# sozoluffy/TensorNetworks

Hardware: AMD Instinct MI355X
Metric: ksd_gradient_steps_per_sec (higher is better)
Workload: dtype f64; 1 GPU; n16_L6_dense; n_qubits=16, layers=6, ansatz=hardware_efficient, params=288, gram=dense, bayesian_network=synthetic n=16 seed=0 (SURVEY 8d), optimizer=adam lr=0.005 cosine clip=10, parallelism=paramshift + gram row shard x1

## Files before the change

tensornetworks_amd/csrc/plan.cpp:

```cpp
#include "plan.hpp"

#include <algorithm>
#include <array>
#include <cstring>
#include <utility>

namespace bornvi {

int num_params(int ansatz, int n, int layers) {
  if (ansatz == 0 || ansatz == 1) return layers * 3 * n;
  if (ansatz == 2) return layers * 2 * n;
  return -1;
}

bool build_gate_list(int ansatz, int n, int layers, std::vector<Gate>& g) {
  g.clear();
  int p = 0;
  auto rot = [&](int kind, int w) { g.push_back({kind, w, -1, p++}); };
  if (ansatz == 0) {
    for (int i = 0; i < n; ++i) g.push_back({G_H, i, -1, -1});
    for (int l = 0; l < layers; ++l) {
      for (int i = 0; i < n; ++i) { rot(G_RX, i); rot(G_RY, i); rot(G_RZ, i); }
      if (n > 1) {
        for (int i = 0; i + 1 < n; ++i) g.push_back({G_CNOT, i, i + 1, -1});
        if (n > 2) g.push_back({G_CNOT, n - 1, 0, -1});
        if (l % 2 == 0 && n > 2)
          for (int i = 0; i < n - 2; i += 2) g.push_back({G_CZ, i, i + 2, -1});
      }
    }
  } else if (ansatz == 1) {
    for (int i = 0; i < n; ++i) g.push_back({G_H, i, -1, -1});
    for (int l = 0; l < layers; ++l) {
      for (int i = 0; i < n; ++i) { rot(G_RX, i); rot(G_RY, i); rot(G_RZ, i); }
      if (n > 1)
        for (int i = 0; i < n; ++i)
          for (int j = i + 1; j < n; ++j) g.push_back({G_CZ, i, j, -1});
    }
  } else if (ansatz == 2) {
    for (int l = 0; l < layers; ++l) {
      for (int i = 0; i < n; ++i) { rot(G_RY, i); rot(G_RZ, i); }
      if (n > 1) {
        for (int i = 0; i + 1 < n; ++i) g.push_back({G_CNOT, i, i + 1, -1});
        if (n > 2) g.push_back({G_CNOT, n - 1, 0, -1});
      }
    }
  } else {
    return false;
  }
  return true;
}

namespace {

enum { K_U1 = 0, K_CX = 1, K_CZ = 2 };
struct Op { int kind, a, b, idx; };
using Fused = std::array<uint32_t, FUSED_WORDS>;

void fuse_gates(const std::vector<Gate>& gates, int n, std::vector<Op>& ops, std::vector<Fused>& fused) {
  std::vector<int> open(n, -1);
  for (const Gate& g : gates) {
    if (g.kind <= G_RZ) {
      int f = open[g.w0];
      if (f < 0 || fused[f][1] >= (uint32_t)FUSED_MAX_ELEMS) {
        Fused nf; nf.fill(0xffffffffu);
        nf[0] = (uint32_t)g.w0; nf[1] = 0;
        fused.push_back(nf);
        f = (int)fused.size() - 1;
        open[g.w0] = f;
        ops.push_back({K_U1, g.w0, -1, f});
      }
      uint32_t e = fused[f][1]++;
      fused[f][2 + 2 * e] = (uint32_t)g.kind;
      fused[f][3 + 2 * e] = (uint32_t)g.param;
    } else {
      open[g.w0] = open[g.w1] = -1;
      ops.push_back({g.kind == G_CNOT ? K_CX : K_CZ, g.w0, g.w1, -1});
    }
  }
}

inline int op_target(const Op& o) { return o.kind == K_U1 ? o.a : (o.kind == K_CX ? o.b : -1); }

void greedy_select(const std::vector<Op>& ops, const std::vector<int>& pool, int n, int cap,
                   std::vector<int>& sel, std::vector<int>& rest, std::vector<int>& targets) {
  std::vector<char> blocked(n, 0), in_t(n, 0);
  sel.clear(); rest.clear(); targets.clear();
  for (int idx : pool) {
    const Op& o = ops[idx];
    bool blk = blocked[o.a] || (o.b >= 0 && blocked[o.b]);
    int t = op_target(o);
    if (!blk && t >= 0 && !in_t[t]) {
      if ((int)targets.size() < cap) { in_t[t] = 1; targets.push_back(t); }
      else blk = true;
    }
    if (blk) {
      blocked[o.a] = 1;
      if (o.b >= 0) blocked[o.b] = 1;
      rest.push_back(idx);
    } else {
      sel.push_back(idx);
    }
  }
}

int fixed_select(const std::vector<Op>& ops, const std::vector<int>& pool, int n, const std::vector<char>& allowed,
                 std::vector<int>& sel, std::vector<int>& rest, std::vector<int>& targets) {
  std::vector<char> blocked(n, 0), in_t(n, 0);
  sel.clear(); rest.clear(); targets.clear();
  int bound_ops = 0;
  for (int idx : pool) {
    const Op& o = ops[idx];
    bool blk = blocked[o.a] || (o.b >= 0 && blocked[o.b]);
    const int t = op_target(o);
    if (!blk && t >= 0 && !allowed[t]) blk = true;
    if (blk) {
      blocked[o.a] = 1;
      if (o.b >= 0) blocked[o.b] = 1;
      rest.push_back(idx);
    } else {
      if (t >= 0) { ++bound_ops; if (!in_t[t]) { in_t[t] = 1; targets.push_back(t); } }
      sel.push_back(idx);
    }
  }
  return bound_ops;
}

void choose_pass(const std::vector<Op>& ops, const std::vector<int>& pool, int n, int k, std::vector<int>& sel,
                 std::vector<int>& rest, std::vector<int>& targets) {
  std::vector<std::vector<char>> cands;
  {
    std::vector<int> s, r, t;
    greedy_select(ops, pool, n, k, s, r, t);
    std::vector<char> a(n, 0);
    for (int w : t) a[w] = 1;
    int cnt = (int)t.size();
    for (int w = n - 1; w >= 0 && cnt < k; --w) if (!a[w]) { a[w] = 1; ++cnt; }
    cands.push_back(a);
  }
  if (k < n)
    for (int s0 = 0; s0 < n; ++s0) {
      std::vector<char> a(n, 0);
      for (int j = 0; j < k; ++j) a[(s0 + j) % n] = 1;
      cands.push_back(a);
    }
  long best_score = -1;
  std::vector<int> s1, r1, t1, s2, r2, t2;
  for (const auto& a : cands) {
    const int here = fixed_select(ops, pool, n, a, s1, r1, t1);
    if (s1.empty()) continue;
    int next_best = 0;
    if (!r1.empty() && k < n)
      for (const auto& a2 : cands) {
        const int nb = fixed_select(ops, r1, n, a2, s2, r2, t2);
        if (nb > next_best) next_best = nb;
      }
    const long score = (long)(here + next_best) * 4096 + (long)s1.size();
    if (score > best_score) { best_score = score; sel = s1; rest = r1; targets = t1; }
  }
  if (best_score < 0) greedy_select(ops, pool, n, k, sel, rest, targets);
}

struct StageSel {
  std::vector<int> pre_cx, pre_cz, us, post_cx, post_cz, targets;
  size_t count() const { return pre_cx.size() + pre_cz.size() + us.size() + post_cx.size() + post_cz.size(); }
};

void stage_select(const std::vector<Op>& ops, const std::vector<int>& pool, int n, int cap, StageSel& S,
                  std::vector<int>& rest, bool defer_cx3 = false, bool read_map = false) {
  std::vector<char> blocked(n, 0), in_t(n, 0), has_u(n, 0);
  std::vector<int> wphase(n, 0);
  rest.clear();
  for (int idx : pool) {
    const Op& o = ops[idx];
    bool blk = blocked[o.a] || (o.b >= 0 && blocked[o.b]);
    int ph = -1;
    if (!blk) {
      const int mx = std::max(wphase[o.a], o.b >= 0 ? wphase[o.b] : 0);
      if (o.kind == K_U1) ph = (mx <= 1 && !has_u[o.a]) ? 2 : -1;
      else if (o.kind == K_CX) ph = mx <= 0 ? 0 : (mx <= 3 ? 3 : -1);
      else ph = mx <= 1 ? 1 : (mx <= 4 ? 4 : -1);
      if (ph < 0) blk = true;
    }
    const int t = op_target(o);
    if (!blk && t >= 0 && !in_t[t] && !(read_map && o.kind == K_CX && ph == 0)) {
      if (defer_cx3 && o.kind == K_CX) blk = true;
      else if ((int)S.targets.size() < cap) { in_t[t] = 1; S.targets.push_back(t); }
      else blk = true;
    }
    if (blk) {
      blocked[o.a] = 1;
      if (o.b >= 0) blocked[o.b] = 1;
      rest.push_back(idx);
      continue;
    }
    wphase[o.a] = std::max(wphase[o.a], ph);
    if (o.b >= 0) wphase[o.b] = std::max(wphase[o.b], ph);
    switch (ph) {
      case 0: S.pre_cx.push_back(idx); break;
      case 1: S.pre_cz.push_back(idx); break;
      case 2: S.us.push_back(idx); has_u[o.a] = 1; break;
      case 3: S.post_cx.push_back(idx); break;
      default: S.post_cz.push_back(idx); break;
    }
  }
}

std::vector<int> order_for_banks(std::vector<int> pos) {
  std::sort(pos.begin(), pos.end());
  std::vector<int> out;
  std::vector<char> used(pos.size(), 0);
  bool res_used[4] = {false, false, false, false};
  auto take = [&](auto pred) -> bool {
    for (size_t i = 0; i < pos.size(); ++i)
      if (!used[i] && pred(pos[i])) { used[i] = 1; out.push_back(pos[i]); res_used[pos[i] & 3] = true; return true; }
    return false;
  };
  for (int s = 0; s < 3 && out.size() < pos.size(); ++s)
    if (!take([&](int p) { return (p & 3) != 3 && !res_used[p & 3]; }))
      take([&](int) { return true; });
  if (out.size() < pos.size())
    if (!take([&](int p) { return (p & 3) == 3; })) take([&](int) { return true; });
  if (out.size() < pos.size() && out.size() >= 2) {
    int r0 = out[0] & 3, r1 = out[1] & 3;
    if (!take([&](int p) { return (p & 3) == r0 || (p & 3) == r1; })) take([&](int) { return true; });
  }
  for (size_t i = 0; i < pos.size(); ++i)
    if (!used[i]) out.push_back(pos[i]);
  return out;
}

void split_pass_ops(const std::vector<Op>& ops, const std::vector<int>& pass_ops, int n, bool is_init,
                    std::vector<int>& lead, std::vector<int>& core, std::vector<int>& trail) {
  lead.clear(); core.clear(); trail.clear();
  std::vector<char> touched(n, 0);
  std::vector<int> mid;
  for (int idx : pass_ops) {
    const Op& o = ops[idx];
    if (!is_init && o.kind == K_CX && !touched[o.a] && !touched[o.b]) { lead.push_back(idx); continue; }
    touched[o.a] = 1; if (o.b >= 0) touched[o.b] = 1;
    mid.push_back(idx);
  }
  std::fill(touched.begin(), touched.end(), 0);
  std::vector<int> trail_rev, core_rev;
  for (size_t q = mid.size(); q-- > 0;) {
    const Op& o = ops[mid[q]];
    if (o.kind == K_CX && !touched[o.a] && !touched[o.b]) { trail_rev.push_back(mid[q]); continue; }
    touched[o.a] = 1; if (o.b >= 0) touched[o.b] = 1;
    core_rev.push_back(mid[q]);
  }
  core.assign(core_rev.rbegin(), core_rev.rend());
  trail.assign(trail_rev.rbegin(), trail_rev.rend());
}

int count_stages(const std::vector<Op>& ops, const std::vector<int>& core, int n, int r, bool defer_cx3, bool read_map) {
  std::vector<int> pool = core, rest;
  int cnt = 0;
  while (!pool.empty()) {
    StageSel sel;
    stage_select(ops, pool, n, r, sel, rest, defer_cx3, read_map);
    if (sel.count() == 0) return 1 << 20;
    ++cnt;
    pool = rest;
  }
  return cnt;
}
bool pick_defer_policy(const std::vector<Op>& ops, const std::vector<int>& core, int n, int r, bool read_map) {
  return read_map && count_stages(ops, core, n, r, true, true) < count_stages(ops, core, n, r, false, true);
}

void first_last_stage_targets(const std::vector<Op>& ops, const std::vector<int>& pass_ops, int n, int r, bool is_init,
                              std::vector<int>& first_t, std::vector<int>& last_t, bool read_map) {
  std::vector<int> lead, core, trail, rest;
  split_pass_ops(ops, pass_ops, n, is_init, lead, core, trail);
  first_t.clear(); last_t.clear();
  std::vector<int> pool = core;
  bool first = true;
  const bool defer = pick_defer_policy(ops, core, n, r, read_map);
  while (!pool.empty()) {
    StageSel sel;
    stage_select(ops, pool, n, r, sel, rest, defer, read_map);
    if (sel.count() == 0) break;
    if (first) { first_t = sel.targets; first = false; }
    last_t = sel.targets;
    pool = rest;
  }
}

struct PassInfo {
  std::vector<int> ops;
  std::vector<int> targets;
  std::vector<int> local;
  std::vector<int> global;
  std::vector<int> lds_wire;
  std::vector<int> in_low;
  std::vector<int> out_low;
};

}

namespace {
struct BuildSpec {
  int n = 0;
  std::vector<Op> ops;
  std::vector<Fused> fused;
  int n_params = 0, n_gates = 0;
  bool in_state = false;
  bool out_state = false;
  std::vector<std::pair<int, int>> out_perm;
};
bool build_plan(const BuildSpec& spec, const PlanOptions& opt, Plan& plan, std::string& msg);
}

namespace {
bool make_plan_impl(int ansatz, int n, int layers, const PlanOptions& opt, Plan& plan, std::string& msg, std::vector<TailOp>* tail);
}

bool make_plan(int ansatz, int n, int layers, const PlanOptions& opt, Plan& plan, std::string& msg) {
  return make_plan_impl(ansatz, n, layers, opt, plan, msg, nullptr);
}

bool make_state_plan(int ansatz, int n, int layers, const PlanOptions& opt, Plan& plan, std::vector<TailOp>& tail, std::string& msg) {
  tail.clear();
  return make_plan_impl(ansatz, n, layers, opt, plan, msg, &tail);
}

namespace {
bool make_plan_impl(int ansatz, int n, int layers, const PlanOptions& opt, Plan& plan, std::string& msg, std::vector<TailOp>* tail) {
  if (n < 1 || n > MAX_PLAN_QUBITS) { msg = "num qubits must be in [1, " + std::to_string(MAX_PLAN_QUBITS) + "]"; return false; }
  if (layers < 0) { msg = "layers must be >= 0"; return false; }
  std::vector<Gate> gates;
  if (!build_gate_list(ansatz, n, layers, gates)) { msg = "unknown ansatz id"; return false; }
  BuildSpec spec;
  spec.n = n;
  fuse_gates(gates, n, spec.ops, spec.fused);
  {
    size_t last_u = spec.ops.size();
    while (last_u > 0 && spec.ops[last_u - 1].kind != K_U1) --last_u;
    for (size_t q = last_u; q < spec.ops.size(); ++q) {
      if (tail) tail->push_back({spec.ops[q].kind == K_CZ ? 1 : 0, spec.ops[q].a, spec.ops[q].b});
      else if (spec.ops[q].kind == K_CX) spec.out_perm.push_back({spec.ops[q].a, spec.ops[q].b});
    }
    spec.ops.resize(last_u);
  }
  spec.out_state = tail != nullptr;
  spec.n_params = num_params(ansatz, n, layers);
  spec.n_gates = (int)gates.size();
  if (opt.kmulti == 0 && n > opt.kmax && opt.kmax >= 13) {
    PlanOptions o11 = opt, o13 = opt;
    o11.kmulti = 11;
    o13.kmulti = 13;
    if (opt.r == 3) return build_plan(spec, o13, plan, msg);
    Plan p13;
    std::string m13;
    if (build_plan(spec, o13, p13, m13)) {
      FastTables ft;
      if ((build_fast_tables(p13, FAST_TABLE_MAX_BYTES, ft) && p13.fast_lds_bytes(ft.max_tab_rows) <= MAX_LDS_BYTES) ||
          n - o11.kmulti > 16) {
        plan = std::move(p13);
        return true;
      }
    }
    return build_plan(spec, o11, plan, msg);
  }
  return build_plan(spec, opt, plan, msg);
}
}

bool make_kron_plan(int n, const PlanOptions& opt, Plan& plan, std::string& msg) {
  if (n < 1 || n > MAX_PLAN_QUBITS) { msg = "num bits must be in [1, " + std::to_string(MAX_PLAN_QUBITS) + "]"; return false; }
  BuildSpec spec;
  spec.n = n;
  Fused f; f.fill(0xffffffffu); f[0] = 0; f[1] = 0;
  spec.fused.push_back(f);
  for (int w = n - 1; w >= 0; --w) spec.ops.push_back({K_U1, w, -1, 0});
  spec.in_state = spec.out_state = true;
  spec.n_gates = n;
  if (opt.kmulti == 0 && n - 12 > 16 && opt.kmax >= 13) {
    PlanOptions o13 = opt;
    o13.kmulti = 13;
    return build_plan(spec, o13, plan, msg);
  }
  return build_plan(spec, opt, plan, msg);
}

namespace {
bool build_plan(const BuildSpec& spec, const PlanOptions& opt, Plan& plan, std::string& msg) {
  const int n = spec.n;
  const std::vector<Op>& ops = spec.ops;
  const std::vector<Fused>& fused = spec.fused;
  const int kmulti = opt.kmulti > 0 ? opt.kmulti : (n <= 16 ? 11 : 12);
  const int k = (n <= opt.kmax) ? n : std::min(opt.kmax, kmulti);
  const int r = std::min(opt.r, k);
  if (r > 4) { msg = "at most 4 register wires"; return false; }
  int threads = 64;
  while (threads < (1 << (k - r))) threads <<= 1;
  if (threads > opt.max_threads) { msg = "tile needs more threads than allowed"; return false; }
  if (fused.size() > 65535) { msg = "too many fused gates"; return false; }

  std::vector<PassInfo> passes;
  {
    std::vector<int> pool(ops.size());
    for (size_t i = 0; i < ops.size(); ++i) pool[i] = (int)i;
    std::vector<int> sel, rest, tg;
    while (!pool.empty()) {
      choose_pass(ops, pool, n, k, sel, rest, tg);
      if (sel.empty()) { msg = "planner made no progress"; return false; }
      PassInfo pi; pi.ops = sel; pi.targets = tg;
      passes.push_back(pi);
      pool = rest;
    }
    if (passes.empty()) passes.push_back(PassInfo{});
  }
  const int lo_can = std::min(opt.lo, k);
  std::vector<int> canon_low;
  for (int p = 0; p < lo_can; ++p) canon_low.push_back(n - 1 - p);
  std::vector<int> canon_low_out = canon_low;
  {
    auto count_with = [&](int lo) {
      std::vector<char> in(n, 0);
      int cnt = 0;
      for (int w : passes.back().targets) { in[w] = 1; ++cnt; }
      for (int p = 0; p < lo; ++p) if (!in[n - 1 - p]) { in[n - 1 - p] = 1; ++cnt; }
      return cnt;
    };
    int lo_fit = -1;
    for (int lo = lo_can; lo >= std::min(3, lo_can); --lo)
      if (count_with(lo) <= k) { lo_fit = lo; break; }
    if (lo_fit < 0) passes.push_back(PassInfo{});
    else canon_low_out.resize(lo_fit);
  }
  if (spec.in_state) {
    std::vector<char> in(n, 0);
    int cnt = 0;
    for (int w : passes.front().targets) { in[w] = 1; ++cnt; }
    for (int w : canon_low) if (!in[w]) { in[w] = 1; ++cnt; }
    if (cnt > k) passes.insert(passes.begin(), PassInfo{});
  }
  const int np = (int)passes.size();
  for (int i = 0; i < np; ++i) {
    PassInfo& P = passes[i];
    std::vector<char> in(n, 0);
    auto add = [&](int w) { if (!in[w] && (int)P.local.size() < k) { in[w] = 1; P.local.push_back(w); } };
    for (int w : P.targets) add(w);
    if (i == np - 1) for (int w : canon_low_out) add(w);
    if (i == 0 && spec.in_state) for (int w : canon_low) add(w);
    if (i + 1 < np) for (int w : passes[i + 1].targets) add(w);
    if (i > 0) for (int w : passes[i - 1].local) add(w);
    for (int w = n - 1; w >= 0; --w) add(w);
    for (int w = 0; w < n; ++w) if (!in[w]) P.global.push_back(w);
  }
  if (spec.in_state) passes[0].in_low = canon_low;
  for (int i = 0; i < np; ++i) {
    PassInfo& P = passes[i];
    std::vector<char> placed(n, 0);
    for (int w : P.in_low) { P.lds_wire.push_back(w); placed[w] = 1; }
    std::vector<int> others;
    for (int w : P.local) if (!placed[w]) others.push_back(w);
    std::sort(others.begin(), others.end());
    for (int w : others) P.lds_wire.push_back(w);
    if (i == np - 1) { P.out_low = canon_low_out; break; }
    std::vector<char> nxt(n, 0);
    for (int w : passes[i + 1].local) nxt[w] = 1;
    std::vector<int> ldspos(n, -1);
    for (int j = 0; j < k; ++j) ldspos[P.lds_wire[j]] = j;
    std::vector<int> pos;
    for (int w : P.local) if (nxt[w]) pos.push_back(ldspos[w]);
    {
      std::vector<int> f_cur, l_cur, f_nxt, l_nxt;
      first_last_stage_targets(ops, P.ops, n, r, i == 0 && !spec.in_state, f_cur, l_cur, opt.use_read_map());
      first_last_stage_targets(ops, passes[i + 1].ops, n, r, false, f_nxt, l_nxt, opt.use_read_map());
      std::vector<char> busy(n, 0);
      for (int w : l_cur) busy[w] = 1;
      for (int w : f_nxt) busy[w] = 1;
      std::vector<int> quiet;
      for (int q : pos) if (!busy[P.lds_wire[q]]) quiet.push_back(q);
      if ((int)quiet.size() >= std::min(4, std::min(opt.lo, k))) pos = quiet;
    }
    pos = order_for_banks(pos);
    const int lo = std::min((int)pos.size(), std::min(opt.lo, k));
    for (int j = 0; j < lo; ++j) P.out_low.push_back(P.lds_wire[pos[j]]);
    passes[i + 1].in_low = P.out_low;
  }
  std::vector<std::vector<int>> layout(np, std::vector<int>(n, -1));
  for (int i = 0; i < np; ++i) {
    if (i == np - 1) { for (int w = 0; w < n; ++w) layout[i][w] = n - 1 - w; continue; }
    int p = 0;
    for (int w : passes[i].out_low) layout[i][w] = p++;
    if (opt.contig_out) {
      std::vector<char> nxt(n, 0);
      for (int w : passes[i + 1].local) nxt[w] = 1;
      for (int w : passes[i].local) if (layout[i][w] < 0 && nxt[w]) layout[i][w] = p++;
      for (int w : passes[i].local) if (layout[i][w] < 0) layout[i][w] = p++;
    }
    for (int w = 0; w < n; ++w) if (layout[i][w] < 0) layout[i][w] = p++;
  }

  std::vector<uint32_t>& W = plan.words;
  plan.max_stages = 0;
  W.assign(PH_SIZE, 0);
  W[PH_MAGIC] = PLAN_MAGIC; W[PH_N] = n; W[PH_K] = k; W[PH_NPASSES] = np;
  W[PH_NFUSED] = (uint32_t)fused.size(); W[PH_NPARAMS] = (uint32_t)spec.n_params;
  W[PH_THREADS] = threads; W[PH_R] = r; W[PH_NGATES] = (uint32_t)spec.n_gates;
  W[PH_OFF_FUSED] = (uint32_t)W.size();
  for (const Fused& f : fused) W.insert(W.end(), f.begin(), f.end());
  W[PH_OFF_PASSTAB] = (uint32_t)W.size();
  W.resize(W.size() + np, 0);
  plan.pass_off.assign(np, 0);

  for (int i = 0; i < np; ++i) {
    const PassInfo& P = passes[i];
    const uint32_t base = (uint32_t)W.size();
    plan.pass_off[i] = base;
    W[W[PH_OFF_PASSTAB] + i] = base;
    W.resize(base + PW_STAGES, 0);
    uint32_t flags = 0;
    if (i == 0 && !spec.in_state) flags |= PASS_INIT;
    if (i == np - 1) flags |= spec.out_state ? PASS_FINAL_STATE : PASS_FINAL;
    std::vector<int> ldspos(n, -1), gpos(n, -1);
    for (int j = 0; j < k; ++j) ldspos[P.lds_wire[j]] = j;
    for (int m = 0; m < n - k; ++m) gpos[P.global[m]] = m;
    auto extpos = [&](int w) { return ldspos[w] >= 0 ? ldspos[w] : k + gpos[w]; };
    const int lo_in = (int)P.in_low.size(), lo_out = (int)P.out_low.size();
    W[base + PW_FLAGS] = flags; W[base + PW_K] = k; W[base + PW_N] = n;
    W[base + PW_LO_IN] = lo_in; W[base + PW_LO_OUT] = lo_out; W[base + PW_THREADS] = threads;
    auto put_byte = [&](int table, int j, int value) { W[base + table + (j >> 2)] |= (uint32_t)value << (8 * (j & 3)); };
    if (k > 16 || n - k > 16) { msg = "tile or workgroup index wider than 16 bits"; return false; }
    for (int j = 0; j < k; ++j) {
      W[base + PW_WIRE_OF_LDS + j] = P.lds_wire[j];
      put_byte(PW_IN_PHYS, j, (i > 0) ? layout[i - 1][P.lds_wire[j]] : (n - 1 - P.lds_wire[j]));
    }
    for (int m = 0; m < n - k; ++m) {
      W[base + PW_WIRE_OF_G + m] = P.global[m];
      put_byte(PW_IN_GPHYS, m, (i > 0) ? layout[i - 1][P.global[m]] : (n - 1 - P.global[m]));
      put_byte(PW_OUT_GPHYS, m, layout[i][P.global[m]]);
    }
    std::vector<int> lead, core, trail;
    split_pass_ops(ops, P.ops, n, (flags & PASS_INIT) != 0, lead, core, trail);
    struct LExpr { uint32_t l, g; };
    auto compose_lin = [&](const std::vector<int>& seq, bool reverse) {
      std::vector<LExpr> ex(k);
      for (int b2 = 0; b2 < k; ++b2) ex[b2] = LExpr{1u << b2, 0u};
      for (size_t q = 0; q < seq.size(); ++q) {
        const Op& o = ops[seq[reverse ? seq.size() - 1 - q : q]];
        const LExpr ce = ldspos[o.a] >= 0 ? ex[ldspos[o.a]] : LExpr{0u, 1u << gpos[o.a]};
        ex[ldspos[o.b]].l ^= ce.l; ex[ldspos[o.b]].g ^= ce.g;
      }
      return ex;
    };
    auto put_half = [&](int table, int j, uint32_t value) { W[base + table + (j >> 1)] |= (value & 0xffffu) << (16 * (j & 1)); };
    {
      const std::vector<LExpr> fin = compose_lin(lead, false);
      for (int j = 0; j < k; ++j) {
        uint32_t col = 0;
        for (int b2 = 0; b2 < k; ++b2) col |= ((fin[b2].l >> j) & 1u) << b2;
        put_half(PW_IN_MASK, j, lds_swizzle(col));
      }
      for (int m = 0; m < n - k; ++m) {
        uint32_t col = 0;
        for (int b2 = 0; b2 < k; ++b2) col |= ((fin[b2].g >> m) & 1u) << b2;
        put_half(PW_IN_GMASK, m, lds_swizzle(col));
      }
    }
    {
      const std::vector<LExpr> fout = compose_lin(trail, true);
      auto out_col = [&](int q) { uint32_t col = 0; for (int b2 = 0; b2 < k; ++b2) col |= ((fout[b2].l >> q) & 1u) << b2; return lds_swizzle(col); };
      std::vector<char> isl(n, 0);
      int j = 0;
      for (int w : P.out_low) { put_half(PW_OUT_MASK, j, out_col(ldspos[w])); put_byte(PW_OUT_PHYS, j, layout[i][w]); isl[w] = 1; ++j; }
      for (int q = 0; q < k; ++q) {
        int w = P.lds_wire[q];
        if (isl[w]) continue;
        put_half(PW_OUT_MASK, j, out_col(q)); put_byte(PW_OUT_PHYS, j, layout[i][w]); ++j;
      }
      for (int m = 0; m < n - k; ++m) {
        uint32_t col = 0;
        for (int b2 = 0; b2 < k; ++b2) col |= ((fout[b2].g >> m) & 1u) << b2;
        put_half(PW_OUT_GMASK, m, lds_swizzle(col));
      }
      std::vector<uint32_t> wire_col(n, 0);
      for (int w = 0; w < n; ++w) wire_col[w] = 1u << layout[i][w];
      if (i == np - 1 && !spec.out_perm.empty()) {
        std::vector<uint32_t> reach(n);
        std::vector<uint32_t> expr(n);
        for (int w = 0; w < n; ++w) expr[w] = 1u << w;
        for (const auto& cx : spec.out_perm) expr[cx.second] ^= expr[cx.first];
        for (int w = 0; w < n; ++w) {
          uint32_t col = 0;
          for (int w2 = 0; w2 < n; ++w2) if ((expr[w2] >> w) & 1u) col ^= 1u << layout[i][w2];
          wire_col[w] = col;
        }
      }
      {
        std::vector<char> isl2(n, 0);
        int j2 = 0;
        for (int w : P.out_low) { W[base + PW_OUT_COL + j2] = wire_col[w]; isl2[w] = 1; ++j2; }
        for (int q = 0; q < k; ++q) {
          const int w = P.lds_wire[q];
          if (isl2[w]) continue;
          W[base + PW_OUT_COL + j2] = wire_col[w]; ++j2;
        }
        for (int m = 0; m < n - k; ++m) W[base + PW_OUT_GCOL + m] = wire_col[P.global[m]];
      }
    }
    std::vector<int> pool = core, rest;
    uint32_t nstages = 0;
    const bool defer_cx3 = pick_defer_policy(ops, core, n, r, opt.use_read_map());
    while (!pool.empty()) {
      StageSel sel;
      stage_select(ops, pool, n, r, sel, rest, defer_cx3, opt.use_read_map());
      if (sel.count() == 0) { msg = "stage planner made no progress"; return false; }
      std::vector<char> isr(n, 0);
      std::vector<int> regw;
      {
        std::vector<char> has_u(n, 0);
        for (int idx : sel.us) has_u[ops[idx].a] = 1;
        for (int w : sel.targets) if (has_u[w]) regw.push_back(w);
        for (int w : sel.targets) if (!has_u[w]) regw.push_back(w);
      }
      for (int w : regw) isr[w] = 1;
      {
        std::vector<char> lowwire(n, 0);
        for (int w : P.in_low) lowwire[w] = 1;
        for (int w : P.out_low) lowwire[w] = 1;
        for (int avoid = 1; avoid >= 0; --avoid)
          for (int j = k - 1; j >= 0 && (int)regw.size() < r; --j)
            if (!isr[P.lds_wire[j]] && !(avoid && lowwire[P.lds_wire[j]])) { isr[P.lds_wire[j]] = 1; regw.push_back(P.lds_wire[j]); }
      }
      std::vector<int> regbit(n, -1);
      uint32_t rho = 0;
      for (int b = 0; b < r; ++b) { regbit[regw[b]] = b; rho |= (uint32_t)ldspos[regw[b]] << (8 * b); }
      std::vector<int> freepos;
      for (int j = 0; j < k; ++j) if (!isr[P.lds_wire[j]]) freepos.push_back(j);
      freepos = order_for_banks(freepos);
      uint32_t io_flags = 0;
      {
        const bool first = (nstages == 0) && !(flags & PASS_INIT);
        const bool last = rest.empty();
        auto lead_with = [&](const std::vector<int>& lowpos) {
          for (int q : lowpos) if (isr[P.lds_wire[q]]) return false;
          std::vector<char> taken(k, 0);
          std::vector<int> others;
          for (int q : lowpos) taken[q] = 1;
          for (int q : freepos) if (!taken[q]) others.push_back(q);
          std::vector<int> ord = lowpos;
          ord.insert(ord.end(), others.begin(), others.end());
          freepos = ord;
          return true;
        };
        if (first && !P.in_low.empty()) {
          std::vector<int> lowpos;
          for (size_t q = 0; q < P.in_low.size(); ++q) lowpos.push_back((int)q);
          if ((int)lowpos.size() <= k - r && lead_with(lowpos)) io_flags |= STAGE_FROM_HBM;
        }
        if (last && !(io_flags & STAGE_FROM_HBM) && !P.out_low.empty()) {
          std::vector<int> lowpos;
          for (int w : P.out_low) lowpos.push_back(ldspos[w]);
          if ((int)lowpos.size() <= k - r && lead_with(lowpos)) io_flags |= STAGE_TO_HBM;
        }
      }
      uint32_t tpos[4] = {0, 0, 0, 0};
      for (size_t j = 0; j < freepos.size() && j < 16; ++j) tpos[j / 4] |= (uint32_t)freepos[j] << (8 * (j % 4));

      struct Expr { uint32_t areg, bext; };
      auto compose = [&](const std::vector<int>& seq, bool reverse, Expr (&ex)[4]) {
        for (int t = 0; t < 4; ++t) ex[t] = Expr{1u << t, 0u};
        for (size_t q = 0; q < seq.size(); ++q) {
          const Op& o = ops[seq[reverse ? seq.size() - 1 - q : q]];
          const int rt = regbit[o.b];
          Expr ce = regbit[o.a] >= 0 ? ex[regbit[o.a]] : Expr{0u, 1u << extpos(o.a)};
          ex[rt].areg ^= ce.areg; ex[rt].bext ^= ce.bext;
        }
      };
      Expr pre[4], post[4];
      compose(sel.post_cx, false, post);
      std::vector<Expr> pre_pos((size_t)k);
      for (int p2 = 0; p2 < k; ++p2) pre_pos[(size_t)p2] = Expr{0u, 1u << p2};
      for (int t = 0; t < r; ++t) pre_pos[(size_t)ldspos[regw[t]]] = Expr{1u << t, 0u};
      for (size_t q = 0; q < sel.pre_cx.size(); ++q) {
        const Op& o = ops[sel.pre_cx[sel.pre_cx.size() - 1 - q]];
        const Expr ce = ldspos[o.a] >= 0 ? pre_pos[(size_t)ldspos[o.a]] : Expr{0u, 1u << extpos(o.a)};
        Expr& te = pre_pos[(size_t)ldspos[o.b]];
        te.areg ^= ce.areg; te.bext ^= ce.bext;
      }
      for (int t = 0; t < 4; ++t) pre[t] = t < r ? pre_pos[(size_t)ldspos[regw[t]]] : Expr{1u << t, 0u};
      auto slot_offset = [&](const Expr (&ex)[4], int j) {
        uint32_t off = 0;
        for (int t = 0; t < r; ++t)
          if (__builtin_popcount(ex[t].areg & (uint32_t)j) & 1) off |= 1u << ldspos[regw[t]];
        return off;
      };
      auto read_slot_offset = [&](int j) {
        uint32_t off = 0;
        for (int p2 = 0; p2 < k; ++p2)
          if (__builtin_popcount(pre_pos[(size_t)p2].areg & (uint32_t)j) & 1) off |= 1u << p2;
        return off;
      };
      auto emit_signq = [&](const std::vector<int>& czs, const Expr (&ex)[4]) {
        uint32_t U[32]; std::memset(U, 0, sizeof(U));
        uint32_t Sym[32]; std::memset(Sym, 0, sizeof(Sym));
        for (int idx : czs) {
          int ea = extpos(ops[idx].a), eb = extpos(ops[idx].b);
          int lo2 = std::min(ea, eb), hi2 = std::max(ea, eb);
          U[lo2] ^= 1u << hi2;
          Sym[lo2] ^= 1u << hi2; Sym[hi2] ^= 1u << lo2;
        }
        for (int a = 0; a < 32; ++a) W.push_back(U[a]);
        uint32_t qbits = 0;
        for (int j = 0; j < 16; ++j) {
          uint32_t off = (j < (1 << r)) ? slot_offset(ex, j) : 0u, m = 0, qv = 0;
          for (int a = 0; a < 32; ++a)
            if (off >> a & 1) { m ^= Sym[a]; qv ^= (uint32_t)__builtin_popcount(off & U[a]) & 1u; }
          W.push_back(m);
          qbits |= qv << j;
        }
        W.push_back(qbits);
      };

      const uint32_t sbase = (uint32_t)W.size();
      W.resize(sbase + STAGE_HDR_WORDS, 0);
      W[sbase + 1] = rho;
      for (int q = 0; q < 4; ++q) W[sbase + 2 + q] = tpos[q];
      uint32_t fidx[4] = {0xffffu, 0xffffu, 0xffffu, 0xffffu};
      for (int idx : sel.us) fidx[regbit[ops[idx].a]] = (uint32_t)ops[idx].idx;
      W[sbase + 6] = fidx[0] | (fidx[1] << 16);
      W[sbase + 7] = fidx[2] | (fidx[3] << 16);
      if (nstages >= (uint32_t)MAX_STAGES) { msg = "too many stages in one pass"; return false; }
      W[base + PW_MATS + 2 * nstages] = W[sbase + 6];
      W[base + PW_MATS + 2 * nstages + 1] = W[sbase + 7];
      for (int t = 0; t < 4; ++t) { W[sbase + 8 + t] = t < r ? pre[t].bext : 0u; W[sbase + 12 + t] = t < r ? post[t].bext : 0u; }
      for (int j = 0; j < 16; ++j) {
        W[sbase + 16 + j] = (j < (1 << r)) ? lds_swizzle(read_slot_offset(j)) : 0u;
        W[sbase + 32 + j] = (j < (1 << r)) ? lds_swizzle(slot_offset(post, j)) : 0u;
      }
      bool cross_read = false;
      for (int p2 = 0; p2 < k; ++p2)
        if (!isr[P.lds_wire[p2]]) {
          W[sbase + 48 + p2] = pre_pos[(size_t)p2].bext ^ (1u << p2);
          if (W[sbase + 48 + p2] || pre_pos[(size_t)p2].areg) cross_read = true;
        }
      uint32_t flags = io_flags | (cross_read ? STAGE_CROSS_READ : 0u);
      Expr ident[4];
      for (int t = 0; t < 4; ++t) ident[t] = Expr{1u << t, 0u};
      if (!sel.pre_cz.empty()) { flags |= STAGE_SIGN_PRE; emit_signq(sel.pre_cz, ident); }
      if (!sel.post_cz.empty()) { flags |= STAGE_SIGN_POST; emit_signq(sel.post_cz, post); }
      for (uint32_t tt = 0; tt < (1u << (k - r)); ++tt) {
        uint32_t bse = 0;
        for (size_t j = 0; j < freepos.size(); ++j) bse |= ((tt >> j) & 1u) << freepos[j];
        W.push_back(lds_swizzle(bse) | (bse << 16));
      }
      const uint32_t nwords = (uint32_t)W.size() - sbase;
      if (nwords >= (1u << 16)) { msg = "stage too large"; return false; }
      W[sbase] = (uint32_t)r | (flags << 8) | (nwords << 16);
      ++nstages;
      pool = rest;
    }
    W[base + PW_NSTAGES] = nstages;
    if ((int)nstages > plan.max_stages) plan.max_stages = (int)nstages;
  }
  W[PH_TOTAL] = (uint32_t)W.size();
  plan.param_first_pass.assign(spec.n_params, np > 0 ? np - 1 : 0);
  std::vector<char> param_seen(spec.n_params, 0);
  for (int i = 0; i < np; ++i) {
    const uint32_t* PWp = W.data() + plan.pass_off[i];
    for (uint32_t sm = 0; sm < PWp[PW_NSTAGES] * 4u; ++sm) {
      const uint32_t w = PWp[PW_MATS + (sm >> 1)];
      const uint32_t f = (sm & 1u) ? (w >> 16) : (w & 0xffffu);
      if (f == 0xffffu) continue;
      const uint32_t* fw = W.data() + W[PH_OFF_FUSED] + f * FUSED_WORDS;
      for (uint32_t e = 0; e < fw[1]; ++e) {
        const uint32_t par = fw[3 + 2 * e];
        if (par != 0xffffffffu && par < (uint32_t)spec.n_params && !param_seen[par]) { param_seen[par] = 1; plan.param_first_pass[par] = i; }
      }
    }
  }
  for (int q = 0; q < spec.n_params; ++q) if (!param_seen[q]) plan.param_first_pass[q] = 0;
  plan.n = n; plan.k = k; plan.r = r; plan.n_passes = np; plan.n_fused = (int)fused.size();
  plan.n_params = spec.n_params; plan.threads = threads; plan.n_gates = spec.n_gates;
  return true;
}
}

bool build_fast_tables(const Plan& plan, size_t max_bytes, FastTables& out) {
  out.words.clear(); out.pass_off.clear(); out.any_sign = false; out.max_tab_rows = 1;
  const int n = plan.n, k = plan.k;
  const int r = plan.r;
  if ((r != 4 && r != 3) || k < (r == 4 ? 10 : 9) || plan.threads != (1 << (k - r)) || n - k > 16) return false;
  out.r = r;
  const int kt = k - r;
  const int nslots = 1 << r;
  const size_t per_stage = (size_t)1 << (n - r);
  size_t total = 0;
  for (int i = 0; i < plan.n_passes; ++i) {
    const uint32_t* P = plan.words.data() + plan.pass_off[i];
    const uint32_t nst = P[PW_NSTAGES];
    if (nst > (uint32_t)MAX_STAGES || nst * 4u * (uint32_t)r > (uint32_t)plan.threads) return false;
    bool any_sign = false;
    const uint32_t* S = P + PW_STAGES;
    for (uint32_t s = 0; s < nst; ++s) { if ((S[0] >> 8) & (STAGE_SIGN_PRE | STAGE_SIGN_POST)) any_sign = true; S += S[0] >> 16; }
    total += FH_WORDS + (size_t)nst * FS_WORDS + (size_t)nst * per_stage * (any_sign ? 2 : 1) + 2 * per_stage;
  }
  if (total * sizeof(uint32_t) > max_bytes || total >= (size_t)0xffffffffu) return false;
  std::vector<uint32_t>& W = out.words;
  W.reserve(total);
  auto parity = [](uint32_t v) { return (uint32_t)__builtin_popcount(v) & 1u; };
  for (int i = 0; i < plan.n_passes; ++i) {
    const uint32_t* P = plan.words.data() + plan.pass_off[i];
    const uint32_t nst = P[PW_NSTAGES];
    const uint32_t hbase = (uint32_t)W.size();
    out.pass_off.push_back(hbase);
    W.resize(hbase + FH_WORDS + (size_t)nst * FS_WORDS, 0);
    uint32_t sign_pre = 0, sign_post = 0;
    {
      const uint32_t* S = P + PW_STAGES;
      for (uint32_t s = 0; s < nst; ++s) {
        const uint32_t sf = (S[0] >> 8) & 0xffu;
        if (sf & STAGE_SIGN_PRE) sign_pre |= 1u << s;
        if (sf & STAGE_SIGN_POST) sign_post |= 1u << s;
        S += S[0] >> 16;
      }
    }
    const bool any_sign = (sign_pre | sign_post) != 0;
    if (any_sign) out.any_sign = true;
    out.max_tab_rows = std::max(out.max_tab_rows, (int)nst + __builtin_popcount(sign_pre | sign_post));
    const uint32_t rw_base = (uint32_t)W.size();
    W.resize(W.size() + (size_t)nst * per_stage, 0);
    const uint32_t sg_base = any_sign ? (uint32_t)W.size() : 0u;
    if (any_sign) W.resize(W.size() + (size_t)nst * per_stage, 0);
    W[hbase + FH_NSTAGES] = nst; W[hbase + FH_RW_BASE] = rw_base; W[hbase + FH_SG_BASE] = sg_base;
    W[hbase + FH_SIGN_PRE] = sign_pre; W[hbase + FH_SIGN_POST] = sign_post;
    const uint32_t* S = P + PW_STAGES;
    for (uint32_t s = 0; s < nst; ++s) {
      const uint32_t hdr = S[0];
      if ((hdr & 0xffu) != (uint32_t)r) { out.words.clear(); out.pass_off.clear(); return false; }
      const uint32_t sflags = (hdr >> 8) & 0xffu, nwords = hdr >> 16, rho = S[1];
      uint32_t* FS = W.data() + hbase + FH_WORDS + (size_t)s * FS_WORDS;
      FS[FS_FI01] = S[6]; FS[FS_FI23] = S[7];
      {
        const uint32_t fi[4] = {S[6] & 0xffffu, S[6] >> 16, S[7] & 0xffffu, S[7] >> 16};
        uint32_t ng = 0;
        while (ng < (uint32_t)r && fi[ng] != 0xffffu) ++ng;
        for (uint32_t b = ng; b < 4; ++b)
          if (fi[b] != 0xffffu) { out.words.clear(); out.pass_off.clear(); return false; }
        FS[FS_KIND] = ng | ((sflags & STAGE_SIGN_PRE) ? 8u : 0u) | ((sflags & STAGE_SIGN_POST) ? 16u : 0u);
        FS[FS_CROSS] = (sflags & STAGE_CROSS_READ) ? 1u : 0u;
        if (!fast_stage_kind_supported(FS[FS_KIND])) { out.words.clear(); out.pass_off.clear(); return false; }
      }
      for (int b = 0; b < r; ++b) { FS[FS_RB + b] = S[16 + (1 << b)] << 4; FS[FS_WB + b] = S[32 + (1 << b)] << 4; }
      for (int j = 0; j < nslots; ++j) {
        uint32_t lr = 0, lw = 0;
        for (int b = 0; b < r; ++b) if (j >> b & 1) { lr ^= S[16 + (1 << b)]; lw ^= S[32 + (1 << b)]; }
        if (lr != S[16 + j] || lw != S[32 + j]) { out.words.clear(); out.pass_off.clear(); return false; }
      }
      uint32_t sri[4] = {0, 0, 0, 0}, rpos[4] = {0, 0, 0, 0};
      for (int b = 0; b < r; ++b) { rpos[b] = (rho >> (8 * b)) & 0xffu; sri[b] = lds_swizzle(1u << rpos[b]); }
      const uint32_t* Qpre = (sflags & STAGE_SIGN_PRE) ? S + STAGE_HDR_WORDS : nullptr;
      const uint32_t* Qpost = (sflags & STAGE_SIGN_POST) ? S + STAGE_HDR_WORDS + (Qpre ? SIGNQ_WORDS : 0) : nullptr;
      const uint32_t* tab = S + STAGE_HDR_WORDS + (Qpre ? SIGNQ_WORDS : 0) + (Qpost ? SIGNQ_WORDS : 0);
      auto sign_bits = [&](const uint32_t* Q, uint32_t e) {
        uint32_t acc = 0;
        for (int q = 0; q < n; ++q) acc ^= ((e >> q) & 1u) & parity(e & Q[q]);
        uint32_t m = 0;
        for (int j = 0; j < 16; ++j) m |= (((Q[48] >> j) ^ acc ^ parity(e & Q[32 + j])) & 1u) << j;
        return m;
      };
      uint32_t* RW = W.data() + rw_base + (size_t)s * per_stage;
      uint32_t* SG = any_sign ? W.data() + sg_base + (size_t)s * per_stage : nullptr;
      for (uint32_t g = 0; g < (1u << (n - k)); ++g)
        for (uint32_t t = 0; t < (1u << kt); ++t) {
          const uint32_t pb = tab[t] & 0xffffu, base = tab[t] >> 16;
          const uint32_t e = base | (g << k);
          uint32_t lflip = 0, sflip = 0, e2 = e;
          for (int b = 0; b < r; ++b) {
            if (parity(e & S[8 + b])) lflip ^= sri[b];
            if (parity(e & S[12 + b])) { sflip ^= sri[b]; e2 |= 1u << rpos[b]; }
          }
          for (int p2 = 0; p2 < k; ++p2)
            if (S[48 + p2] && parity(e & S[48 + p2])) lflip ^= lds_swizzle(1u << p2);
          RW[((size_t)g << kt) + t] = (pb ^ lflip) | ((pb ^ sflip) << 16);
          if (SG) SG[((size_t)g << kt) + t] = (Qpre ? sign_bits(Qpre, e) : 0u) | ((Qpost ? sign_bits(Qpost, e2) : 0u) << 16);
        }
      S += nwords;
    }
    const uint32_t pflags = P[PW_FLAGS];
    const uint32_t kt2 = (uint32_t)kt;
    auto tbyte = [&](int table, int j) { return (P[table + (j >> 2)] >> (8 * (j & 3))) & 0xffu; };
    auto thalf = [&](int table, int j) { return (P[table + (j >> 1)] >> (16 * (j & 1))) & 0xffffu; };
    const uint32_t ksize = 1u << k;
    const uint32_t ngl = 1u << (n - k);
    if (nst > 0) {
      const uint32_t* S0 = P + PW_STAGES;
      const uint32_t* SL = S0;
      for (uint32_t s2 = 0; s2 + 1 < nst; ++s2) SL += SL[0] >> 16;
      const uint32_t f0 = (S0[0] >> 8) & 0xffu, fl = (SL[0] >> 8) & 0xffu;
      std::vector<uint32_t> inv(ksize);
      if ((f0 & STAGE_FROM_HBM) && !(pflags & PASS_INIT)) {
        auto slot_lin = [&](uint32_t u) { uint32_t o = 0; for (int j = 0; j < k; ++j) if (u >> j & 1) o ^= thalf(PW_IN_MASK, j); return o; };
        auto phys_u = [&](uint32_t u) { uint32_t o = 0; for (int j = 0; j < k; ++j) if (u >> j & 1) o |= 1u << tbyte(PW_IN_PHYS, j); return o; };
        for (uint32_t u = 0; u < ksize; ++u) inv[slot_lin(u)] = u;
        const uint32_t tab = (uint32_t)W.size();
        W.resize(W.size() + per_stage, 0);
        const uint32_t* RW0 = W.data() + rw_base;
        bool ok = true;
        uint32_t basis[4] = {0, 0, 0, 0};
        for (int b = 0; b < r; ++b) basis[b] = phys_u(inv[W[hbase + FH_WORDS + FS_RB + b] >> 4]) << 4;
        for (uint32_t g = 0; g < ngl && ok; ++g) {
          uint32_t gslot = 0, gphys = 0;
          for (int m = 0; m < n - k; ++m) if (g >> m & 1) { gslot ^= thalf(PW_IN_GMASK, m); gphys |= 1u << tbyte(PW_IN_GPHYS, m); }
          for (uint32_t t = 0; t < (1u << kt2); ++t) {
            const uint32_t rslot = RW0[((size_t)g << kt2) + t] & 0xffffu;
            const uint32_t off = (phys_u(inv[rslot ^ gslot]) | gphys) << 4;
            W[tab + ((size_t)g << kt2) + t] = off;
          }
// ... 398 lines not shown
```

Before: 236.1 steps/s.

## Let the pass and stage planners commute gates that share diagonal (control/CZ) wires

```diff
diff --git a/tensornetworks_amd/csrc/plan.cpp b/tensornetworks_amd/csrc/plan.cpp
--- a/tensornetworks_amd/csrc/plan.cpp
+++ b/tensornetworks_amd/csrc/plan.cpp
@@ -81,21 +81,31 @@
 
 inline int op_target(const Op& o) { return o.kind == K_U1 ? o.a : (o.kind == K_CX ? o.b : -1); }
 
-void greedy_select(const std::vector<Op>& ops, const std::vector<int>& pool, int n, int cap,
+enum : char { BLOCK_DIAG = 1, BLOCK_FULL = 2 };
+inline bool acts_diagonally(const Op& o, int w) { return o.kind == K_CZ || (o.kind == K_CX && w == o.a); }
+inline bool held_back(const Op& o, const std::vector<char>& blocked, bool commute) {
+  auto held = [&](int w) { return w >= 0 && (blocked[w] == BLOCK_FULL || (blocked[w] == BLOCK_DIAG && !(commute && acts_diagonally(o, w)))); };
+  return held(o.a) || held(o.b);
+}
+inline void block_wires(const Op& o, std::vector<char>& blocked) {
+  auto block = [&](int w) { if (w >= 0) blocked[w] = std::max<char>(blocked[w], acts_diagonally(o, w) ? BLOCK_DIAG : BLOCK_FULL); };
+  block(o.a); block(o.b);
+}
+
+void greedy_select(const std::vector<Op>& ops, const std::vector<int>& pool, int n, int cap, bool commute,
                    std::vector<int>& sel, std::vector<int>& rest, std::vector<int>& targets) {
   std::vector<char> blocked(n, 0), in_t(n, 0);
   sel.clear(); rest.clear(); targets.clear();
   for (int idx : pool) {
     const Op& o = ops[idx];
-    bool blk = blocked[o.a] || (o.b >= 0 && blocked[o.b]);
+    bool blk = held_back(o, blocked, commute);
     int t = op_target(o);
     if (!blk && t >= 0 && !in_t[t]) {
       if ((int)targets.size() < cap) { in_t[t] = 1; targets.push_back(t); }
       else blk = true;
     }
     if (blk) {
-      blocked[o.a] = 1;
-      if (o.b >= 0) blocked[o.b] = 1;
+      block_wires(o, blocked);
       rest.push_back(idx);
     } else {
       sel.push_back(idx);
@@ -103,19 +113,18 @@
   }
 }
 
-int fixed_select(const std::vector<Op>& ops, const std::vector<int>& pool, int n, const std::vector<char>& allowed,
+int fixed_select(const std::vector<Op>& ops, const std::vector<int>& pool, int n, const std::vector<char>& allowed, bool commute,
                  std::vector<int>& sel, std::vector<int>& rest, std::vector<int>& targets) {
   std::vector<char> blocked(n, 0), in_t(n, 0);
   sel.clear(); rest.clear(); targets.clear();
   int bound_ops = 0;
   for (int idx : pool) {
     const Op& o = ops[idx];
-    bool blk = blocked[o.a] || (o.b >= 0 && blocked[o.b]);
+    bool blk = held_back(o, blocked, commute);
     const int t = op_target(o);
     if (!blk && t >= 0 && !allowed[t]) blk = true;
     if (blk) {
-      blocked[o.a] = 1;
-      if (o.b >= 0) blocked[o.b] = 1;
+      block_wires(o, blocked);
       rest.push_back(idx);
     } else {
       if (t >= 0) { ++bound_ops; if (!in_t[t]) { in_t[t] = 1; targets.push_back(t); } }
@@ -125,12 +134,12 @@
   return bound_ops;
 }
 
-void choose_pass(const std::vector<Op>& ops, const std::vector<int>& pool, int n, int k, std::vector<int>& sel,
+void choose_pass(const std::vector<Op>& ops, const std::vector<int>& pool, int n, int k, bool commute, std::vector<int>& sel,
                  std::vector<int>& rest, std::vector<int>& targets) {
   std::vector<std::vector<char>> cands;
   {
     std::vector<int> s, r, t;
-    greedy_select(ops, pool, n, k, s, r, t);
+    greedy_select(ops, pool, n, k, commute, s, r, t);
     std::vector<char> a(n, 0);
     for (int w : t) a[w] = 1;
     int cnt = (int)t.size();
@@ -146,18 +155,18 @@
   long best_score = -1;
   std::vector<int> s1, r1, t1, s2, r2, t2;
   for (const auto& a : cands) {
-    const int here = fixed_select(ops, pool, n, a, s1, r1, t1);
+    const int here = fixed_select(ops, pool, n, a, commute, s1, r1, t1);
     if (s1.empty()) continue;
     int next_best = 0;
     if (!r1.empty() && k < n)
       for (const auto& a2 : cands) {
-        const int nb = fixed_select(ops, r1, n, a2, s2, r2, t2);
+        const int nb = fixed_select(ops, r1, n, a2, commute, s2, r2, t2);
         if (nb > next_best) next_best = nb;
       }
     const long score = (long)(here + next_best) * 4096 + (long)s1.size();
     if (score > best_score) { best_score = score; sel = s1; rest = r1; targets = t1; }
   }
-  if (best_score < 0) greedy_select(ops, pool, n, k, sel, rest, targets);
+  if (best_score < 0) greedy_select(ops, pool, n, k, commute, sel, rest, targets);
 }
 
 struct StageSel {
@@ -165,14 +174,14 @@
   size_t count() const { return pre_cx.size() + pre_cz.size() + us.size() + post_cx.size() + post_cz.size(); }
 };
 
-void stage_select(const std::vector<Op>& ops, const std::vector<int>& pool, int n, int cap, StageSel& S,
+void stage_select(const std::vector<Op>& ops, const std::vector<int>& pool, int n, int cap, bool commute, StageSel& S,
                   std::vector<int>& rest, bool defer_cx3 = false, bool read_map = false) {
   std::vector<char> blocked(n, 0), in_t(n, 0), has_u(n, 0);
   std::vector<int> wphase(n, 0);
   rest.clear();
   for (int idx : pool) {
     const Op& o = ops[idx];
-    bool blk = blocked[o.a] || (o.b >= 0 && blocked[o.b]);
+    bool blk = held_back(o, blocked, commute);
     int ph = -1;
     if (!blk) {
       const int mx = std::max(wphase[o.a], o.b >= 0 ? wphase[o.b] : 0);
@@ -188,8 +197,7 @@
       else blk = true;
     }
     if (blk) {
-      blocked[o.a] = 1;
-      if (o.b >= 0) blocked[o.b] = 1;
+      block_wires(o, blocked);
       rest.push_back(idx);
       continue;
     }
@@ -252,33 +260,33 @@
   trail.assign(trail_rev.rbegin(), trail_rev.rend());
 }
 
-int count_stages(const std::vector<Op>& ops, const std::vector<int>& core, int n, int r, bool defer_cx3, bool read_map) {
+int count_stages(const std::vector<Op>& ops, const std::vector<int>& core, int n, int r, bool commute, bool defer_cx3, bool read_map) {
   std::vector<int> pool = core, rest;
   int cnt = 0;
   while (!pool.empty()) {
     StageSel sel;
-    stage_select(ops, pool, n, r, sel, rest, defer_cx3, read_map);
+    stage_select(ops, pool, n, r, commute, sel, rest, defer_cx3, read_map);
     if (sel.count() == 0) return 1 << 20;
     ++cnt;
     pool = rest;
   }
   return cnt;
 }
-bool pick_defer_policy(const std::vector<Op>& ops, const std::vector<int>& core, int n, int r, bool read_map) {
-  return read_map && count_stages(ops, core, n, r, true, true) < count_stages(ops, core, n, r, false, true);
-}
-
-void first_last_stage_targets(const std::vector<Op>& ops, const std::vector<int>& pass_ops, int n, int r, bool is_init,
+bool pick_defer_policy(const std::vector<Op>& ops, const std::vector<int>& core, int n, int r, bool commute, bool read_map) {
+  return read_map && count_stages(ops, core, n, r, commute, true, true) < count_stages(ops, core, n, r, commute, false, true);
+}
+
+void first_last_stage_targets(const std::vector<Op>& ops, const std::vector<int>& pass_ops, int n, int r, bool is_init, bool commute,
                               std::vector<int>& first_t, std::vector<int>& last_t, bool read_map) {
   std::vector<int> lead, core, trail, rest;
   split_pass_ops(ops, pass_ops, n, is_init, lead, core, trail);
   first_t.clear(); last_t.clear();
   std::vector<int> pool = core;
   bool first = true;
-  const bool defer = pick_defer_policy(ops, core, n, r, read_map);
+  const bool defer = pick_defer_policy(ops, core, n, r, commute, read_map);
   while (!pool.empty()) {
     StageSel sel;
-    stage_select(ops, pool, n, r, sel, rest, defer, read_map);
+    stage_select(ops, pool, n, r, commute, sel, rest, defer, read_map);
     if (sel.count() == 0) break;
     if (first) { first_t = sel.targets; first = false; }
     last_t = sel.targets;
@@ -308,7 +316,7 @@
   bool out_state = false;
   std::vector<std::pair<int, int>> out_perm;
 };
-bool build_plan(const BuildSpec& spec, const PlanOptions& opt, Plan& plan, std::string& msg);
+bool build_plan(const BuildSpec& spec, const PlanOptions& opt, bool may_commute, Plan& plan, std::string& msg);
 }
 
 namespace {
@@ -345,14 +353,15 @@
   spec.out_state = tail != nullptr;
   spec.n_params = num_params(ansatz, n, layers);
   spec.n_gates = (int)gates.size();
+  const bool own_tile = opt.kmulti == 0;
   if (opt.kmulti == 0 && n > opt.kmax && opt.kmax >= 13) {
     PlanOptions o11 = opt, o13 = opt;
     o11.kmulti = 11;
     o13.kmulti = 13;
-    if (opt.r == 3) return build_plan(spec, o13, plan, msg);
+    if (opt.r == 3) return build_plan(spec, o13, own_tile, plan, msg);
     Plan p13;
     std::string m13;
-    if (build_plan(spec, o13, p13, m13)) {
+    if (build_plan(spec, o13, own_tile, p13, m13)) {
       FastTables ft;
       if ((build_fast_tables(p13, FAST_TABLE_MAX_BYTES, ft) && p13.fast_lds_bytes(ft.max_tab_rows) <= MAX_LDS_BYTES) ||
           n - o11.kmulti > 16) {
@@ -360,9 +369,9 @@
         return true;
       }
     }
-    return build_plan(spec, o11, plan, msg);
-  }
-  return build_plan(spec, opt, plan, msg);
+    return build_plan(spec, o11, own_tile, plan, msg);
+  }
+  return build_plan(spec, opt, own_tile, plan, msg);
 }
 }
 
@@ -378,13 +387,38 @@
   if (opt.kmulti == 0 && n - 12 > 16 && opt.kmax >= 13) {
     PlanOptions o13 = opt;
     o13.kmulti = 13;
-    return build_plan(spec, o13, plan, msg);
-  }
-  return build_plan(spec, opt, plan, msg);
+    return build_plan(spec, o13, false, plan, msg);
+  }
+  return build_plan(spec, opt, false, plan, msg);
 }
 
 namespace {
-bool build_plan(const BuildSpec& spec, const PlanOptions& opt, Plan& plan, std::string& msg) {
+bool build_plan_under(const BuildSpec& spec, const PlanOptions& opt, bool commute, Plan& plan, std::string& msg);
+
+std::array<long, 3> plan_cost(const Plan& p) {
+  long stages = 0, first = 0;
+  for (int i = 0; i < p.n_passes; ++i) {
+    const uint32_t* P = p.words.data() + p.pass_off[i];
+    stages += P[PW_NSTAGES];
+    if (i == 0 && (P[PW_FLAGS] & PASS_INIT) && p.n_passes > 1) first = P[PW_NSTAGES];
+  }
+  return {p.n_passes, stages, stages - first};
+}
+
+bool build_plan(const BuildSpec& spec, const PlanOptions& opt, bool may_commute, Plan& plan, std::string& msg) {
+  const bool ok = build_plan_under(spec, opt, false, plan, msg);
+  bool two_qubit = false;
+  for (const Op& o : spec.ops) two_qubit |= o.kind != K_U1;
+  if (!may_commute || !two_qubit) return ok;
+  Plan pc;
+  std::string mc;
+  if (!build_plan_under(spec, opt, true, pc, mc)) return ok;
+  const std::array<long, 3> cc = plan_cost(pc), c0 = ok ? plan_cost(plan) : cc;
+  if (!ok || (cc < c0 && cc[1] <= c0[1])) { plan = std::move(pc); msg.clear(); }
+  return true;
+}
+
+bool build_plan_under(const BuildSpec& spec, const PlanOptions& opt, bool commute, Plan& plan, std::string& msg) {
   const int n = spec.n;
   const std::vector<Op>& ops = spec.ops;
   const std::vector<Fused>& fused = spec.fused;
@@ -403,7 +437,7 @@
     for (size_t i = 0; i < ops.size(); ++i) pool[i] = (int)i;
     std::vector<int> sel, rest, tg;
     while (!pool.empty()) {
-      choose_pass(ops, pool, n, k, sel, rest, tg);
+      choose_pass(ops, pool, n, k, commute, sel, rest, tg);
       if (sel.empty()) { msg = "planner made no progress"; return false; }
       PassInfo pi; pi.ops = sel; pi.targets = tg;
       passes.push_back(pi);
@@ -467,8 +501,8 @@
     for (int w : P.local) if (nxt[w]) pos.push_back(ldspos[w]);
     {
       std::vector<int> f_cur, l_cur, f_nxt, l_nxt;
-      first_last_stage_targets(ops, P.ops, n, r, i == 0 && !spec.in_state, f_cur, l_cur, opt.use_read_map());
-      first_last_stage_targets(ops, passes[i + 1].ops, n, r, false, f_nxt, l_nxt, opt.use_read_map());
+      first_last_stage_targets(ops, P.ops, n, r, i == 0 && !spec.in_state, commute, f_cur, l_cur, opt.use_read_map());
+      first_last_stage_targets(ops, passes[i + 1].ops, n, r, false, commute, f_nxt, l_nxt, opt.use_read_map());
       std::vector<char> busy(n, 0);
       for (int w : l_cur) busy[w] = 1;
       for (int w : f_nxt) busy[w] = 1;
@@ -604,10 +638,10 @@
     }
     std::vector<int> pool = core, rest;
     uint32_t nstages = 0;
-    const bool defer_cx3 = pick_defer_policy(ops, core, n, r, opt.use_read_map());
+    const bool defer_cx3 = pick_defer_policy(ops, core, n, r, commute, opt.use_read_map());
     while (!pool.empty()) {
       StageSel sel;
-      stage_select(ops, pool, n, r, sel, rest, defer_cx3, opt.use_read_map());
+      stage_select(ops, pool, n, r, commute, sel, rest, defer_cx3, opt.use_read_map());
       if (sel.count() == 0) { msg = "stage planner made no progress"; return false; }
       std::vector<char> isr(n, 0);
       std::vector<int> regw;
```

Result: faster. 240.2 steps/s (median of 6 runs) (+1.7%).
